# Gaurav14cs17/Bayer_Low_light_Image_Enhancement

Measured on AMD Instinct MI355X. Metric: megapixels/sec RawFormer-S 512x512 RAW->sRGB, higher is better.
Workload: dtype f32; 1 GPU; RawFormer-S(FLCA) dim=32, batch=8 of packed 4x512x512 synthetic Bayer per GPU; frames_per_gpu=8, variant=flca, weights=synthetic (seeded, random-init scale), parallelism=batch-sharded x1, device=AMD Radeon Graphics

## Files before the change

### bayer_low_light_image_enhancement_amd/build.py

```python
from __future__ import annotations

import os
import shutil
import subprocess
import sys
import tempfile
from concurrent.futures import ThreadPoolExecutor

HERE = os.path.dirname(os.path.abspath(__file__))
CSRC = os.path.join(HERE, "csrc")
LIB = os.path.join(CSRC, "librawformer_hip.so")
DIAG_LIB = os.path.join(CSRC, "librawformer_hip_diag.so")
DIAG_SOURCES = ["rf_block.hip", "rf_model.hip", "rf_gemm1x1.hip", "rf_fused.hip"]
SOURCES = ["rf_api.hip", "rf_registry.hip", "rf_model.hip", "rf_pack.hip", "rf_pointwise.hip", "rf_gemm1x1.hip",
           "rf_conv3x3.hip", "rf_attn.hip", "rf_flca.hip", "rf_fused.hip", "rf_fused_tail.hip", "rf_block.hip", "rf_harness.hip", "rf_ssim.hip", "rf_tokattn.hip", "rf_wfb.hip", "rf_upcat.hip", "rf_fft.hip", "rf_ffab.hip", "rf_truecolor.hip", "rf_multilvl.hip", "rf_train.hip", "rf_trainstep.hip", "rf_sampler.hip", "rf_mamba.hip", "rf_mamba_bwd.hip", "rf_wmb.hip"]
HEADERS = [os.path.join(CSRC, "rf_common.h"), os.path.join(CSRC, "rf_handle.h"), os.path.join(CSRC, "rf_fused_tile.h"), os.path.join(CSRC, "rf_mamba.h"), os.path.join(HERE, "..", "include", "rawformer_hip.h"),
           os.path.join(HERE, "isa_check.py")]
FLAGS = ["-O3", "-std=c++17", "-fPIC", "--offload-arch=gfx950", "-Wall", "-Wno-unused-function"]


def _hipcc() -> str:
    exe = shutil.which("hipcc") or "/opt/rocm/bin/hipcc"
    if not os.path.exists(exe):
        raise RuntimeError("hipcc not found: the RawFormer HIP library cannot be built here")
    return exe


def _run(cmd, cwd=None) -> str:
    r = subprocess.run(cmd, capture_output=True, text=True, cwd=cwd)
    if r.returncode != 0:
        raise RuntimeError("build step failed:\n" + " ".join(cmd) + "\n" + r.stdout + r.stderr)
    return r.stderr


def compile_source(src: str, obj: str, extra_flags=(), verbose: bool = False) -> int:
    from . import isa_check

    hipcc = _hipcc()
    llvm = isa_check.LLVM_BIN
    flags = [*FLAGS, *extra_flags]
    tmp = tempfile.mkdtemp(prefix="rf_build_")
    try:
        dev_s, dev_o, dev_co, fb = (os.path.join(tmp, n) for n in ("dev.s", "dev.o", "dev.co", "dev.hipfb"))
        warn = _run([hipcc, *flags, "--cuda-device-only", "-S", src, "-o", dev_s])
        text, nfix = isa_check.commute_vulnerable(open(dev_s).read())
        if nfix:
            open(dev_s, "w").write(text)
        _run([os.path.join(llvm, "clang"), "-target", "amdgcn-amd-amdhsa", "-mcpu=gfx950", "-c", dev_s, "-o", dev_o])
# ... 63 lines not shown
```

### bayer_low_light_image_enhancement_amd/csrc/rf_attn.hip

```cpp
#include "rf_common.h"

namespace rf {

static constexpr int kMaxBand = 4;
static constexpr int kRowW = kMaxBand * 16 + 2;

__host__ __device__ static inline void band_of(int tq, int C, int c, int* tklo, int* nb) {
    const int lo_ch = 16 * tq;
    const int hi_ch = (16 * tq + 15 < C - 1) ? 16 * tq + 15 : C - 1;
    const int hlo = lo_ch / c, hhi = hi_ch / c;
    const int klo = hlo * c, khi = (hhi + 1) * c - 1;
    *tklo = klo / 16;
    *nb = khi / 16 - *tklo + 1;
}

int gram_plan(int B, int C, int heads, int P, int* nslab, int* slab, size_t* partial_floats) {
    RF_CHECK_ARG(heads > 0 && C % heads == 0, "chan_attn: C=%d not divisible by heads=%d", C, heads);
    const int c = C / heads;
    RF_CHECK_ARG(c <= 64, "chan_attn: head size %d > 64 not supported", c);
    const int NTq = cdiv(C, 16);
    for (int tq = 0; tq < NTq; ++tq) {
        int tklo, nb;
        band_of(tq, C, c, &tklo, &nb);
        RF_CHECK_ARG(nb <= kMaxBand, "chan_attn: C=%d with %d heads (head size %d) needs %d key tiles per query tile, at most %d supported",
// ... 126 lines not shown
    nq += __shfl_xor(nq, 16); nq += __shfl_xor(nq, 32);
    nk += __shfl_xor(nk, 16); nk += __shfl_xor(nk, 32);
#pragma unroll
    for (int r = 0; r < 4; ++r) {
        const int row = 4 * kq + r;
#pragma unroll
        for (int t = 0; t < kMaxBand; ++t) red[wave][row][t * 16 + i] = g[t][r];
        if (row == i) {
            red[wave][row][kMaxBand * 16] = nq;
            red[wave][row][kMaxBand * 16 + 1] = nk;
        }
    }
    __syncthreads();
    float* dst = a.partial + (((size_t)b * a.nslab + slab_id) * gridDim.y + tq) * 16 * kRowW;
    for (int idx = threadIdx.x; idx < 16 * kRowW; idx += 256) {
        const int row = idx / kRowW, col = idx % kRowW;
        dst[idx] = ((red[0][row][col] + red[1][row][col]) + red[2][row][col]) + red[3][row][col];
    }
}

int launch_gram(const GramArgs& a, hipStream_t st) {
    RF_CHECK_ARG(a.B > 0 && a.B <= 65535 && a.C > 0 && a.P > 0, "gram: bad sizes");
    const int vec = (a.P % 4 == 0) && aligned16(a.q) && aligned16(a.k) && (a.bstride % 4 == 0);
    dim3 grid((unsigned)a.nslab, (unsigned)cdiv(a.C, 16), (unsigned)a.B);
    const double c = (double)a.C / a.heads;
    ProfScope prof(st, "gram_kernel", 2.0 * a.C * c * a.P * a.B, 8.0 * a.C * (double)a.P * a.B);
    RF_CHECK_ARG(a.x_hi == 0 || (a.w > 0 && a.P % a.w == 0 && a.x_lo >= 0 && a.x_lo < a.x_hi && a.x_hi <= a.w),
                 "gram: columns [%d, %d) outside the %d-wide image", a.x_lo, a.x_hi, a.w);
    if (a.x_hi > 0) gram_kernel<true><<<grid, 256, 0, st>>>(a, vec);
    else gram_kernel<false><<<grid, 256, 0, st>>>(a, vec);
    return check_launch("gram");
}

__global__ void __launch_bounds__(256) attn_fold_kernel(const float* __restrict__ partial, int nslab,
                                                        const float* __restrict__ temperature,
                                                        const float* __restrict__ w_out, float* __restrict__ wp_out,
                                                        unsigned short* __restrict__ wp3_out, int C, int heads, int log_temperature) {
    const int hd = blockIdx.x, b = blockIdx.y;
    const int c = C / heads;
    const int NT = (C + 15) >> 4;
    __shared__ float S[64][65];
    __shared__ float nq[64], nk[64];
    const float* pb = partial + (size_t)b * nslab * NT * 16 * kRowW;
    __shared__ float sub[256];
    const int nval = c * c + 2 * c;
    int RS = 256 / nval;
    if (RS < 1) RS = 1;
    if (RS > 16) RS = 16;
    for (int base = 0; base < nval; base += 256 / RS) {
        const int vi = base + threadIdx.x / RS, rs = threadIdx.x % RS;
        float s = 0.f;
        if (vi < nval && threadIdx.x / RS < 256 / RS) {
            int qch, col;
            if (vi < c * c) {
                const int ii = vi / c, jj = vi % c;
                qch = hd * c + ii;
                const int kch = hd * c + jj;
                int tklo, nb;
                band_of(qch >> 4, C, c, &tklo, &nb);
                col = ((kch >> 4) - tklo) * 16 + (kch & 15);
            } else if (vi < c * c + c) {
                qch = hd * c + (vi - c * c);
                col = kMaxBand * 16;
            } else {
                qch = hd * c + (vi - c * c - c);
                col = kMaxBand * 16 + 1;
            }
            const float* src = pb + ((size_t)(qch >> 4) * 16 + (qch & 15)) * kRowW + col;
            int sl = rs;
            for (; sl + 7 * RS < nslab; sl += 8 * RS) {
                float t[8];
#pragma unroll
                for (int u = 0; u < 8; ++u) t[u] = src[(size_t)(sl + u * RS) * NT * 16 * kRowW];
#pragma unroll
                for (int u = 0; u < 8; ++u) s += t[u];
            }
            for (; sl < nslab; sl += RS) s += src[(size_t)sl * NT * 16 * kRowW];
        }
        sub[threadIdx.x] = s;
        __syncthreads();
        if (rs == 0 && vi < nval && threadIdx.x / RS < 256 / RS) {
            float t = 0.f;
            for (int q = 0; q < RS; ++q) t += sub[threadIdx.x + q];
            if (vi < c * c) S[vi / c][vi % c] = t;
            else if (vi < c * c + c) nq[vi - c * c] = t;
            else nk[vi - c * c - c] = t;
        }
        __syncthreads();
    }
    if (threadIdx.x < c) {
        const int ii = threadIdx.x;
        const float T = log_temperature ? expf(temperature[hd]) : temperature[hd];
        const float rq = 1.0f / fmaxf(sqrtf(nq[ii]), 1e-12f);
        float m = -INFINITY;
        for (int jj = 0; jj < c; ++jj) {
            const float v = S[ii][jj] * rq * (1.0f / fmaxf(sqrtf(nk[jj]), 1e-12f)) * T;
            S[ii][jj] = v;
            m = fmaxf(m, v);
        }
        float sum = 0.f;
        for (int jj = 0; jj < c; ++jj) {
            const float e = expf(S[ii][jj] - m);
            S[ii][jj] = e;
            sum += e;
        }
        const float inv = 1.0f / sum;
        for (int jj = 0; jj < c; ++jj) S[ii][jj] *= inv;
    }
    __syncthreads();
    float* dst = wp_out + (size_t)b * NT * (C / 4) * 64;
    const int NB = (C + 31) >> 5;
    unsigned short* dst3 = wp3_out ? wp3_out + (size_t)b * NT * NB * 1536 : nullptr;
    for (int idx = threadIdx.x; idx < NT * 16 * c; idx += 256) {
        const int co = idx / c, jj = idx % c;
        float s = 0.f;
        if (co < C) {
            const float* wr = w_out + (size_t)co * C + hd * c;
            for (int ii = 0; ii < c; ++ii) s = fmaf(wr[ii], S[ii][jj], s);
        }
        const int k = hd * c + jj;
        dst[((size_t)(k >> 2) * NT + (co >> 4)) * 64 + (co & 15) + 16 * (k & 3)] = s;
        if (dst3) b3_store(dst3, NT, co, k, s);
    }
    if (dst3 && hd == heads - 1)
        for (int idx = threadIdx.x; idx < NT * 16 * (32 * NB - C); idx += 256)
            b3_store(dst3, NT, idx / (32 * NB - C), C + idx % (32 * NB - C), 0.f);
}

int launch_attn_fold(const float* partial, int nslab, const float* temperature, const float* w_out,
                     float* wp_out, void* wp3_out, int B, int C, int heads, hipStream_t st, int log_temperature) {
    RF_CHECK_ARG(C % heads == 0 && C / heads <= 64 && C % 4 == 0, "attn_fold: unsupported C=%d heads=%d", C, heads);
    ProfScope prof(st, "attn_fold_kernel", 0.0, 0.0);
    attn_fold_kernel<<<dim3((unsigned)heads, (unsigned)B), 256, 0, st>>>(partial, nslab, temperature, w_out, wp_out, (unsigned short*)wp3_out, C, heads, log_temperature);
    return check_launch("attn_fold");
}

}
```

### bayer_low_light_image_enhancement_amd/csrc/rf_fused.hip

```cpp
#include <cstdio>
#include <cstdlib>
#include "rf_common.h"
#ifdef RF_STAMP
namespace rf { __device__ unsigned long long g_stamp[16]; }
#endif
#include "rf_fused_tile.h"

namespace rf {

template <int C, int KP>
__device__ __forceinline__ void load_step_b3p(const float* __restrict__ xb, int P, int kq, const GroupGeom& g, float4 (&xh)[KP / 4]) {
#pragma unroll
    for (int s = 0; s < KP / 4; ++s) {
        const int ch = 32 * (s >> 3) + 8 * kq + (s & 7);
        xh[s] = *reinterpret_cast<const float4*>(xb + (size_t)(ch < C ? ch : 0) * P + (unsigned)g.goff);
    }
}

template <int C, int KP>
__device__ __forceinline__ void ln_step_b3p(int kq, const float* __restrict__ gam_l, const float* __restrict__ bet_l, float eps, float4 (&xh)[KP / 4]) {
    constexpr int NS = KP / 4;
    float sum[4] = {0.f, 0.f, 0.f, 0.f};
#pragma unroll
    for (int s = 0; s < NS; ++s) {
// ... 284 lines not shown
                    const int hc = 4 * s + kq, cv = 2 * C + vp * PART + hc;
                    float v[4];
                    stencil4<Edge::Dpp>(mid + hc * PSV + wave * HC + 4 * j + 4, ro, j, wd_l + cv * 9, bd_l[cv], v);
                    *reinterpret_cast<float4*>(vb + (unsigned)((vp * PART + hc) * P + yo * w + xo)) = make_float4(v[0], v[1], v[2], v[3]);
                }
            }
            STAMP(4);
        }
    }
    STAMP_FLUSH;
    __syncthreads();
    float* red = mid;
#pragma unroll
    for (int r = 0; r < NQT; ++r) {
        for (int i = tid; i < 64 * 48; i += 256) red[(i / 48) * ROWW + 16 + i % 48] = 0.f;
        float nqt = nq[r], nkt = nk[r];
        nqt += __shfl_xor(nqt, 16); nqt += __shfl_xor(nqt, 32);
        nkt += __shfl_xor(nkt, 16); nkt += __shfl_xor(nkt, 32);
#pragma unroll
        for (int q = 0; q < 4; ++q) {
            const int row = 4 * kq + q;
            float* rr = red + (wave * 16 + row) * ROWW;
            rr[j] = gq[r][q];
            if (row == j) { rr[64] = nqt; rr[65] = nkt; }
        }
        __syncthreads();
        float* dst = a.partial + (((size_t)b * a.nslab + slab) * NQT + r) * 16 * ROWW;
        for (int i = tid; i < 16 * ROWW; i += 256)
            dst[i] = ((red[i] + red[16 * ROWW + i]) + red[2 * 16 * ROWW + i]) + red[3 * 16 * ROWW + i];
        __syncthreads();
    }
}

static bool heads_fit_tiles(int C, int heads) {
    const int c = heads > 0 ? C / heads : 0;
    return heads > 0 && C % heads == 0 && c <= 16 && 16 % c == 0;
}
static bool attn_front_shape_ok(int C, int h, int w) { return C == 32 && (w % 4 == 0) && ((double)C * h * w * 4.0 < 4.0e9); }
bool fused_attn_supported(int C, int heads, int h, int w) { return heads_fit_tiles(C, heads) && attn_front_shape_ok(C, h, w); }

int fused_attn_plan(int h, int w, int* nslab, size_t* partial_floats, int B, int C) {
    const int ntiles = cdiv(w, fused::TW) * cdiv(h, fused::TH);
    int ns = cdiv(ntiles, 4);
    if (ntiles <= 256) ns = ntiles;
    if (ns < 1) ns = 1;
    *nslab = ns;
    *partial_floats = (size_t)B * ns * (C / 16) * 16 * 66;
    return RF_OK;
}

int launch_attn_front(AttnFrontArgs a, int C, hipStream_t st) {
    const int B = a.B, h = a.h, w = a.w;
    RF_CHECK_ARG(attn_front_shape_ok(C, h, w) && B <= 65535, "attn_front: unsupported shape C=%d %dx%d", C, h, w);
    RF_CHECK_ARG(aligned16(a.x) && aligned16(a.v), "attn_front: buffers must be 16-byte aligned");
    a.tiles_x = cdiv(w, fused::TW);
    a.ntiles = a.tiles_x * cdiv(h, fused::TH);
    if (!(a.yhi > 0 && a.yhi < h)) a.yhi = h;
    if (!(a.xhi > 0 && a.xhi < w)) a.xhi = w;
    const double px = (double)B * h * w;
    ProfScope prof(st, "attn_front_kernel<32>", px * (6.0 * C * C + 54.0 * C + 4.0 * C * 16), px * 8.0 * C);
    const dim3 grid((unsigned)a.nslab, (unsigned)B);
    attn_front_kernel<32><<<grid, 256, 0, st>>>(a);
    return check_launch("attn_front");
}

template <int C>
__global__ void __launch_bounds__(256, 2) attn_mid_kernel(AttnMidArgs a) {
    using namespace fused;
    constexpr int NQT = C / 16;
    constexpr int NVP = C / PART;
    constexpr int NR = NQT + NVP;
    constexpr int PSG = fused::PSG, PSV = 448, ROWW = 4 * 16 + 2;
    constexpr int NF4 = PART * HR * (HC / 4);
    constexpr int FPT = (NF4 + 255) / 256;
    constexpr unsigned OOB = 0x80000000u;
    __shared__ __attribute__((aligned(16))) float mid[PART * PSG + 8];
    __shared__ float wd_l[3 * C * 9], bd_l[3 * C];

    const int tid = threadIdx.x, lane = tid & 63, wave = tid >> 6;
    const int j = lane & 15, kq = lane >> 4;
    const int slab = blockIdx.x, b = blockIdx.y;
    const int h = a.h, w = a.w, P = h * w;
    const float* qb = a.qkv + (size_t)b * 3 * C * P;
    float* vb = a.v + (size_t)b * C * P;
    for (int i = tid; i < 3 * C * 9; i += 256) wd_l[i] = a.wd[i];
    for (int i = tid; i < 3 * C; i += 256) bd_l[i] = a.bd[i];

    int pk[FPT];
#pragma unroll
    for (int i = 0; i < FPT; ++i) {
        const int e = tid + 256 * i;
        const int pl = e / (HR * (HC / 4)), rem = e % (HR * (HC / 4));
        pk[i] = e < NF4 ? (pl << 16) | ((rem / (HC / 4)) << 8) | (rem % (HC / 4)) : -1;
    }
    const int tiles_y = a.ntiles / a.tiles_x;
    const int per = (a.ntiles + a.nslab - 1) / a.nslab;
    unsigned voff[FPT];
    int pend_ys = 0;
    bool pend_full = true;
    auto plan_tile = [&](int tile, bool full) {
        const int2 o = tile_origin(tile, tiles_y);
        const int x0 = o.x, y0 = o.y;
        pend_ys = y0 % HR; pend_full = full;
#pragma unroll
        for (int i = 0; i < FPT; ++i) {
            int e = pk[i];
            asm volatile("" : "+v"(e));
            const int r = (e >> 8) & 255;
            const int y = y0 - 1 + r, x = x0 - 4 + 4 * (e & 255);
            const bool ok = e >= 0 && (full || r >= 2) && (unsigned)y < (unsigned)h && (unsigned)x < (unsigned)w;
            voff[i] = ok ? (unsigned)((y * w + x) * 4) : OOB;
        }
    };
    float4 stg[FPT];
    auto load_round = [&](int rd) {
        const bool gram = rd < NQT;
        const size_t base = gram ? (size_t)16 * rd * P : (size_t)(2 * C + PART * (rd - NQT)) * P;
        const size_t span = (gram ? (size_t)(C + 16) : (size_t)PART) * P, rest = (size_t)3 * C * P - base;
        const __amdgpu_buffer_rsrc_t rs = __builtin_amdgcn_make_buffer_rsrc(
            const_cast<float*>(qb) + base, 0, (int)((span < rest ? span : rest) * 4), 0x00020000);
        const unsigned kjump = gram ? (unsigned)((C - 16) * P) * 4u : 0u;
#pragma unroll
        for (int i = 0; i < FPT; ++i) {
            const int pl = pk[i] >> 16;
            const unsigned off = voff[i] + (unsigned)pl * (unsigned)P * 4u + (pl >= 16 ? kjump : 0u);
            typedef unsigned u32x4_t __attribute__((ext_vector_type(4)));
            const u32x4_t v4 = __builtin_amdgcn_raw_buffer_load_b128(rs, (int)off, 0, 0);
            stg[i] = make_float4(__uint_as_float(v4.x), __uint_as_float(v4.y), __uint_as_float(v4.z), __uint_as_float(v4.w));
        }
    };
    auto store_round = [&](int rd) {
        const int PSX = rd < NQT ? PSG : PSV;
#pragma unroll
        for (int i = 0; i < FPT; ++i) {
            int e = pk[i];
            asm volatile("" : "+v"(e));
            const int r = (e >> 8) & 255;
            const int slot = pend_ys + r - (pend_ys + r >= HR ? HR : 0);
            if (e >= 0 && (pend_full || r >= 2)) *reinterpret_cast<float4*>(mid + (e >> 16) * PSX + slot * HC + 4 * (e & 255)) = stg[i];
        }
    };

    const int t_begin = slab * per;
    if (t_begin >= a.ntiles) {
        if ((int)blockIdx.z == 0)
            for (int i = tid; i < NQT * 16 * ROWW; i += 256) a.partial[((size_t)b * a.nslab + slab) * NQT * 16 * ROWW + i] = 0.f;
        return;
    }
    const int ntw = (t_begin + per < a.ntiles) ? per : a.ntiles - t_begin;
    f32x4 gq = {0.f, 0.f, 0.f, 0.f};
    float nq = 0.f, nk = 0.f;
    const int rd_lo = (int)blockIdx.z * NR / a.rgroups, rd_hi = ((int)blockIdx.z + 1) * NR / a.rgroups;
    plan_tile(t_begin, true);
    load_round(rd_lo);
    __syncthreads();
    for (int rd = rd_lo; rd < rd_hi; ++rd) {
        for (int ti = 0; ti < ntw; ++ti) {
            const int tile = t_begin + ti;
            const int2 o = tile_origin(tile, tiles_y);
            const int x0 = o.x, y0 = o.y;
            const int yo = y0 + wave;
            lds_barrier();
            store_round(rd);
            int ro[3];
#pragma unroll
            for (int dy = 0; dy < 3; ++dy) {
                const int sl = pend_ys + wave + dy;
                ro[dy] = (sl - (sl >= HR ? HR : 0)) * HC;
            }
            if (ti + 1 < ntw) {
                plan_tile(tile + 1, (tile + 1) % tiles_y == 0);
                load_round(rd);
            } else if (rd + 1 < rd_hi) {
                plan_tile(t_begin, true);
                load_round(rd + 1);
            }
            lds_barrier();
            if (rd < NQT) {
                const int cq = 16 * rd + j, ck = C + 16 * rd + j;
#pragma unroll 1
                for (int st = 0; st < 4; ++st) {
                    const int xo = x0 + 16 * st + 4 * kq;
                    const bool ok = yo >= a.ylo && yo < a.yhi && xo >= a.xlo && xo < a.xhi;
                    float qa[4], kb[4];
                    stencil4<Edge::Wide>(mid + j * PSG + 16 * st + 4 * kq + 4, ro, j, wd_l + cq * 9, bd_l[cq], qa);
                    stencil4<Edge::Wide>(mid + (16 + j) * PSG + 16 * st + 4 * kq + 4, ro, j, wd_l + ck * 9, bd_l[ck], kb);
#pragma unroll
                    for (int m = 0; m < 4; ++m) {
                        const float qv = ok ? qa[m] : 0.f, kv = ok ? kb[m] : 0.f;
                        gq = __builtin_amdgcn_mfma_f32_16x16x4f32(qv, kv, gq, 0, 0, 0);
                        nq = fmaf(qv, qv, nq);
                        nk = fmaf(kv, kv, nk);
                    }
                }
            } else {
                const int vp = rd - NQT, xo = x0 + 4 * j;
                if (yo < h && xo < w) {
#pragma unroll
                    for (int s = 0; s < PART / 4; ++s) {
                        const int hc = 4 * s + kq, cv = 2 * C + vp * PART + hc;
                        float v[4];
                        stencil4<Edge::Dpp>(mid + hc * PSV + 4 * j + 4, ro, j, wd_l + cv * 9, bd_l[cv], v);
                        *reinterpret_cast<float4*>(vb + (size_t)(vp * PART + hc) * P + (size_t)yo * w + xo) = make_float4(v[0], v[1], v[2], v[3]);
                    }
                }
            }
        }
        if (rd < NQT) {
            __syncthreads();
            float* red = mid;
            for (int i = tid; i < 64 * 48; i += 256) red[(i / 48) * ROWW + 16 + i % 48] = 0.f;
            int kq_ = kq;
            asm volatile("" : "+v"(kq_));
            float nqt = nq, nkt = nk;
            nqt += __shfl_xor(nqt, 16); nqt += __shfl_xor(nqt, 32);
            nkt += __shfl_xor(nkt, 16); nkt += __shfl_xor(nkt, 32);
#pragma unroll
            for (int q = 0; q < 4; ++q) {
                const int row = 4 * kq_ + q;
                float* rr = red + (wave * 16 + row) * ROWW;
                rr[j] = gq[q];
                if (row == j) { rr[64] = nqt; rr[65] = nkt; }
            }
            __syncthreads();
            float* dst = a.partial + (((size_t)b * a.nslab + slab) * NQT + rd) * 16 * ROWW;
            for (int i = tid; i < 16 * ROWW; i += 256)
                dst[i] = ((red[i] + red[16 * ROWW + i]) + red[2 * 16 * ROWW + i]) + red[3 * 16 * ROWW + i];
            gq = (f32x4){0.f, 0.f, 0.f, 0.f}; nq = 0.f; nk = 0.f;
        }
    }
}

int attn_mid_plan(int h, int w, int* nslab, size_t* partial_floats, int B, int C) {
    const int ntiles = cdiv(w, fused::TW) * cdiv(h, fused::TH);
    int per = ntiles / 64;
    if (per < 1) per = 1;
    if (per > 8) per = 8;
    *nslab = cdiv(ntiles, per);
    *partial_floats = (size_t)B * *nslab * (C / 16) * 16 * 66;
    return RF_OK;
}

static bool attn_mid_shape_ok(int C, int h, int w) {
    return (C == 64 || C == 128) && (w % 4 == 0) && ((double)(C + 16) * h * w * 4.0 < 2.0e9);
}
bool attn_mid_supported(int C, int heads, int h, int w) { return heads_fit_tiles(C, heads) && attn_mid_shape_ok(C, h, w); }

int launch_attn_mid(AttnMidArgs a, int C, hipStream_t st) {
    const int B = a.B, h = a.h, w = a.w;
    RF_CHECK_ARG(attn_mid_shape_ok(C, h, w) && B <= 65535, "attn_mid: unsupported shape C=%d %dx%d", C, h, w);
    RF_CHECK_ARG(aligned16(a.qkv) && aligned16(a.v), "attn_mid: buffers must be 16-byte aligned");
    a.tiles_x = cdiv(w, fused::TW);
    a.ntiles = a.tiles_x * cdiv(h, fused::TH);
    if (!(a.yhi > 0 && a.yhi < h)) a.yhi = h;
    if (!(a.xhi > 0 && a.xhi < w)) a.xhi = w;
    a.rgroups = ((long)a.nslab * B < 256) ? 3 : 1;
    const double px = (double)B * h * w;
    ProfScope prof(st, C == 64 ? "attn_mid_kernel<64>" : "attn_mid_kernel<128>", px * (54.0 * C + 4.0 * C * 16), px * 16.0 * C);
    const dim3 grid((unsigned)a.nslab, (unsigned)B, (unsigned)a.rgroups);
    if (C == 64) attn_mid_kernel<64><<<grid, 256, 0, st>>>(a);
    else attn_mid_kernel<128><<<grid, 256, 0, st>>>(a);
    return check_launch("attn_mid");
}

#ifdef RF_STAMP
extern "C" int rf_debug_stamps(unsigned long long* out8) {
    unsigned long long z[16] = {0};
    if (hipMemcpyFromSymbol(out8, HIP_SYMBOL(g_stamp), 8 * sizeof(unsigned long long)) != hipSuccess) return -1;
    return hipMemcpyToSymbol(HIP_SYMBOL(g_stamp), z, sizeof(z)) == hipSuccess ? 0 : -1;
}
#endif

}
```

### bayer_low_light_image_enhancement_amd/csrc/rf_fused_tile.h

```cpp
#pragma once
#include "rf_common.h"

namespace rf {

#ifdef RF_STAMP
#define STAMP_DECL unsigned long long st_prev = __builtin_amdgcn_s_memtime(), st_acc[8] = {0, 0, 0, 0, 0, 0, 0, 0};
#define STAMP(i) do { __builtin_amdgcn_sched_barrier(0); unsigned long long t_ = __builtin_amdgcn_s_memtime(); st_acc[i] += t_ - st_prev; st_prev = t_; __builtin_amdgcn_sched_barrier(0); } while (0)
#define STAMP_FLUSH do { if ((threadIdx.x & 63) == 0) for (int i_ = 0; i_ < 8; ++i_) atomicAdd(&g_stamp[i_], st_acc[i_]); } while (0)
#else
#define STAMP_DECL
#define STAMP(i)
#define STAMP_FLUSH
#endif

__device__ __forceinline__ void lds_barrier() {
    asm volatile("s_waitcnt lgkmcnt(0)" ::: "memory");
    __builtin_amdgcn_s_barrier();
    asm volatile("" ::: "memory");
}

namespace fused {
constexpr int TH = 4, TW = 64;
constexpr int HR = TH + 2;
constexpr int HC = 72;
constexpr int NG = HR * (HC / 4);
constexpr int GPW = NG / 4;
constexpr int GPW8 = 14;
constexpr int PART = 32;
constexpr int PSG = 456;
}

struct GroupGeom {
    int lds_off;
    int goff;
    bool valid;
};
template <int G>
__device__ __forceinline__ GroupGeom group_geom(int wave, int st, int j, int y0, int x0, int h, int w) {
    using namespace fused;
    GroupGeom g;
    const int gi = wave * G + st * 16 + j;
    const bool in_step = j < G - st * 16 && (NG % G == 0 || gi < NG);
    const int row = gi / (HC / 4), cg = gi % (HC / 4);
    const int y = y0 - 1 + row, x = x0 - 4 + 4 * cg;
    g.valid = in_step && y >= 0 && y < h && x >= 0 && x < w;
    g.lds_off = in_step ? row * HC + 4 * cg : -1;
    g.goff = g.valid ? y * w + x : 0;
    return g;
}

struct TileRange { int tiles_y, begin, end; };
// ... 292 lines not shown
```

Baseline: 1093 MP/s.

## Move attn_mid to its own file with column-major tile walk and rewrite attn_fold

Moves the attention-mid kernel into its own source file and reworks its tile iteration. Tiles now advance down columns with a rolling row ring in LDS, so each step loads only the new rows, and per-lane load offsets are precomputed once using buffer out-of-bounds masking. Depthwise weights are hoisted per round. The fold kernel may now launch with 1024 threads, unrolls the slab reduction 16-wide, and stages w_out rows in dynamic shared memory. This adds complexity and register pressure in the mid kernel.

```diff
diff --git a/bayer_low_light_image_enhancement_amd/build.py b/bayer_low_light_image_enhancement_amd/build.py
--- a/bayer_low_light_image_enhancement_amd/build.py
+++ b/bayer_low_light_image_enhancement_amd/build.py
@@ -13,7 +13,7 @@
 DIAG_LIB = os.path.join(CSRC, "librawformer_hip_diag.so")
 DIAG_SOURCES = ["rf_block.hip", "rf_model.hip", "rf_gemm1x1.hip", "rf_fused.hip"]
 SOURCES = ["rf_api.hip", "rf_registry.hip", "rf_model.hip", "rf_pack.hip", "rf_pointwise.hip", "rf_gemm1x1.hip",
-           "rf_conv3x3.hip", "rf_attn.hip", "rf_flca.hip", "rf_fused.hip", "rf_fused_tail.hip", "rf_block.hip", "rf_harness.hip", "rf_ssim.hip", "rf_tokattn.hip", "rf_wfb.hip", "rf_upcat.hip", "rf_fft.hip", "rf_ffab.hip", "rf_truecolor.hip", "rf_multilvl.hip", "rf_train.hip", "rf_trainstep.hip", "rf_sampler.hip", "rf_mamba.hip", "rf_mamba_bwd.hip", "rf_wmb.hip"]
+           "rf_conv3x3.hip", "rf_attn.hip", "rf_flca.hip", "rf_fused.hip", "rf_fused_tail.hip", "rf_attn_mid.hip", "rf_block.hip", "rf_harness.hip", "rf_ssim.hip", "rf_tokattn.hip", "rf_wfb.hip", "rf_upcat.hip", "rf_fft.hip", "rf_ffab.hip", "rf_truecolor.hip", "rf_multilvl.hip", "rf_train.hip", "rf_trainstep.hip", "rf_sampler.hip", "rf_mamba.hip", "rf_mamba_bwd.hip", "rf_wmb.hip"]
 HEADERS = [os.path.join(CSRC, "rf_common.h"), os.path.join(CSRC, "rf_handle.h"), os.path.join(CSRC, "rf_fused_tile.h"), os.path.join(CSRC, "rf_mamba.h"), os.path.join(HERE, "..", "include", "rawformer_hip.h"),
            os.path.join(HERE, "isa_check.py")]
 FLAGS = ["-O3", "-std=c++17", "-fPIC", "--offload-arch=gfx950", "-Wall", "-Wno-unused-function"]
diff --git a/bayer_low_light_image_enhancement_amd/csrc/rf_attn.hip b/bayer_low_light_image_enhancement_amd/csrc/rf_attn.hip
--- a/bayer_low_light_image_enhancement_amd/csrc/rf_attn.hip
+++ b/bayer_low_light_image_enhancement_amd/csrc/rf_attn.hip
@@ -182,25 +182,33 @@
     return check_launch("gram");
 }
 
-__global__ void __launch_bounds__(256) attn_fold_kernel(const float* __restrict__ partial, int nslab,
-                                                        const float* __restrict__ temperature,
-                                                        const float* __restrict__ w_out, float* __restrict__ wp_out,
-                                                        unsigned short* __restrict__ wp3_out, int C, int heads, int log_temperature) {
+constexpr int kFoldThreads = 1024;
+constexpr int kFoldStage = 8192;
+static int fold_threads(int c) { return c * c + 2 * c > 256 ? kFoldThreads : 256; }
+__host__ __device__ static inline int fold_stage(int NT, int c) { return NT * 16 * c < kFoldStage ? NT * 16 * c : kFoldStage; }
+__global__ void __launch_bounds__(kFoldThreads) attn_fold_kernel(const float* __restrict__ partial, int nslab,
+                                                                 const float* __restrict__ temperature,
+                                                                 const float* __restrict__ w_out, float* __restrict__ wp_out,
+                                                                 unsigned short* __restrict__ wp3_out, int C, int heads, int log_temperature) {
     const int hd = blockIdx.x, b = blockIdx.y;
     const int c = C / heads;
     const int NT = (C + 15) >> 4;
     __shared__ float S[64][65];
     __shared__ float nq[64], nk[64];
     const float* pb = partial + (size_t)b * nslab * NT * 16 * kRowW;
-    __shared__ float sub[256];
+    extern __shared__ float fold_dyn[];
+    const int nthr = (int)blockDim.x;
+    float* sub = fold_dyn;
     const int nval = c * c + 2 * c;
     int RS = 256 / nval;
     if (RS < 1) RS = 1;
     if (RS > 16) RS = 16;
-    for (int base = 0; base < nval; base += 256 / RS) {
+    const int vpp = nthr / RS;
+    for (int base = 0; base < nval; base += vpp) {
         const int vi = base + threadIdx.x / RS, rs = threadIdx.x % RS;
+        const bool mine = vi < nval && (int)threadIdx.x / RS < vpp;
         float s = 0.f;
-        if (vi < nval && threadIdx.x / RS < 256 / RS) {
+        if (mine) {
             int qch, col;
             if (vi < c * c) {
                 const int ii = vi / c, jj = vi % c;
@@ -217,19 +225,27 @@
                 col = kMaxBand * 16 + 1;
             }
             const float* src = pb + ((size_t)(qch >> 4) * 16 + (qch & 15)) * kRowW + col;
+            const size_t sstride = (size_t)NT * 16 * kRowW;
             int sl = rs;
-            for (; sl + 7 * RS < nslab; sl += 8 * RS) {
-                float t[8];
-#pragma unroll
-                for (int u = 0; u < 8; ++u) t[u] = src[(size_t)(sl + u * RS) * NT * 16 * kRowW];
-#pragma unroll
-                for (int u = 0; u < 8; ++u) s += t[u];
-            }
-            for (; sl < nslab; sl += RS) s += src[(size_t)sl * NT * 16 * kRowW];
+            for (; sl + 15 * RS < nslab; sl += 16 * RS) {
+                float t[16];
+#pragma unroll
+                for (int u = 0; u < 16; ++u) t[u] = src[(size_t)(sl + u * RS) * sstride];
+#pragma unroll
+                for (int u = 0; u < 16; ++u) s += t[u];
+            }
+            for (; sl + 3 * RS < nslab; sl += 4 * RS) {
+                float t[4];
+#pragma unroll
+                for (int u = 0; u < 4; ++u) t[u] = src[(size_t)(sl + u * RS) * sstride];
+#pragma unroll
+                for (int u = 0; u < 4; ++u) s += t[u];
+            }
+            for (; sl < nslab; sl += RS) s += src[(size_t)sl * sstride];
         }
         sub[threadIdx.x] = s;
         __syncthreads();
-        if (rs == 0 && vi < nval && threadIdx.x / RS < 256 / RS) {
+        if (rs == 0 && mine) {
             float t = 0.f;
             for (int q = 0; q < RS; ++q) t += sub[threadIdx.x + q];
             if (vi < c * c) S[vi / c][vi % c] = t;
@@ -261,19 +277,30 @@
     float* dst = wp_out + (size_t)b * NT * (C / 4) * 64;
     const int NB = (C + 31) >> 5;
     unsigned short* dst3 = wp3_out ? wp3_out + (size_t)b * NT * NB * 1536 : nullptr;
-    for (int idx = threadIdx.x; idx < NT * 16 * c; idx += 256) {
-        const int co = idx / c, jj = idx % c;
-        float s = 0.f;
-        if (co < C) {
-            const float* wr = w_out + (size_t)co * C + hd * c;
-            for (int ii = 0; ii < c; ++ii) s = fmaf(wr[ii], S[ii][jj], s);
-        }
-        const int k = hd * c + jj;
-        dst[((size_t)(k >> 2) * NT + (co >> 4)) * 64 + (co & 15) + 16 * (k & 3)] = s;
-        if (dst3) b3_store(dst3, NT, co, k, s);
+    float* wl = fold_dyn + nthr;
+    const int rows = fold_stage(NT, c) / c;
+    for (int co0 = 0; co0 < NT * 16; co0 += rows) {
+        const int nrow = NT * 16 - co0 < rows ? NT * 16 - co0 : rows;
+        __syncthreads();
+        for (int idx = threadIdx.x; idx < nrow * c; idx += nthr) {
+            const int co = co0 + idx / c;
+            wl[idx] = co < C ? w_out[(size_t)co * C + hd * c + idx % c] : 0.f;
+        }
+        __syncthreads();
+        for (int idx = threadIdx.x; idx < nrow * c; idx += nthr) {
+            const int co = co0 + idx / c, jj = idx % c;
+            float s = 0.f;
+            if (co < C) {
+                const float* wr = wl + (idx - jj);
+                for (int ii = 0; ii < c; ++ii) s = fmaf(wr[ii], S[ii][jj], s);
+            }
+            const int k = hd * c + jj;
+            dst[((size_t)(k >> 2) * NT + (co >> 4)) * 64 + (co & 15) + 16 * (k & 3)] = s;
+            if (dst3) b3_store(dst3, NT, co, k, s);
+        }
     }
     if (dst3 && hd == heads - 1)
-        for (int idx = threadIdx.x; idx < NT * 16 * (32 * NB - C); idx += 256)
+        for (int idx = threadIdx.x; idx < NT * 16 * (32 * NB - C); idx += nthr)
             b3_store(dst3, NT, idx / (32 * NB - C), C + idx % (32 * NB - C), 0.f);
 }
 
@@ -281,7 +308,8 @@
                      float* wp_out, void* wp3_out, int B, int C, int heads, hipStream_t st, int log_temperature) {
     RF_CHECK_ARG(C % heads == 0 && C / heads <= 64 && C % 4 == 0, "attn_fold: unsupported C=%d heads=%d", C, heads);
     ProfScope prof(st, "attn_fold_kernel", 0.0, 0.0);
-    attn_fold_kernel<<<dim3((unsigned)heads, (unsigned)B), 256, 0, st>>>(partial, nslab, temperature, w_out, wp_out, (unsigned short*)wp3_out, C, heads, log_temperature);
+    const int c = C / heads, nthr = fold_threads(c);
+    attn_fold_kernel<<<dim3((unsigned)heads, (unsigned)B), nthr, (size_t)(nthr + fold_stage((C + 15) >> 4, c)) * sizeof(float), st>>>(partial, nslab, temperature, w_out, wp_out, (unsigned short*)wp3_out, C, heads, log_temperature);
     return check_launch("attn_fold");
 }
 
diff --git a/bayer_low_light_image_enhancement_amd/csrc/rf_attn_mid.hip b/bayer_low_light_image_enhancement_amd/csrc/rf_attn_mid.hip
--- /dev/null
+++ b/bayer_low_light_image_enhancement_amd/csrc/rf_attn_mid.hip
@@ -0,0 +1,285 @@
+#include <cstdio>
+#include <cstdlib>
+#include "rf_common.h"
+#include "rf_fused_tile.h"
+
+namespace rf {
+
+template <int C>
+__global__ void __launch_bounds__(256, 2) attn_mid_kernel(AttnMidArgs a) {
+    using namespace fused;
+    constexpr int NQT = C / 16;
+    constexpr int NVP = C / PART;
+    constexpr int NR = NQT + NVP;
+    constexpr int PSG = fused::PSG, PSV = 448, ROWW = 4 * 16 + 2;
+    constexpr int G4 = HC / 4;
+    constexpr int PE = PART * 2 * G4;
+    constexpr int KP = (PE + 255) / 256;
+    static_assert(PE == 4 * 256 + 128 && KP == 5, "the last element of a pair belongs to waves 0 and 1");
+    constexpr unsigned OOB = 0x80000000u;
+    __shared__ __attribute__((aligned(16))) float mid[PART * PSG + 8];
+    __shared__ float wd_l[3 * C * 9], bd_l[3 * C];
+
+    const int tid = threadIdx.x, lane = tid & 63, wave = tid >> 6;
+    const int j = lane & 15, kq = lane >> 4;
+    const int slab = blockIdx.x, b = blockIdx.y;
+    const int h = a.h, w = a.w, P = h * w;
+    const float* qb = a.qkv + (size_t)b * 3 * C * P;
+    float* vb = a.v + (size_t)b * C * P;
+    for (int i = tid; i < 3 * C * 9; i += 256) wd_l[i] = a.wd[i];
+    for (int i = tid; i < 3 * C; i += 256) bd_l[i] = a.bd[i];
+
+    const int tiles_y = a.ntiles / a.tiles_x;
+    const int per = (a.ntiles + a.nslab - 1) / a.nslab;
+    const int t_begin = slab * per;
+    if (t_begin >= a.ntiles) {
+        if ((int)blockIdx.z == 0)
+            for (int i = tid; i < NQT * 16 * ROWW; i += 256) a.partial[((size_t)b * a.nslab + slab) * NQT * 16 * ROWW + i] = 0.f;
+        return;
+    }
+    const int ntw = (t_begin + per < a.ntiles) ? per : a.ntiles - t_begin;
+    const int rd_lo = (int)blockIdx.z * NR / a.rgroups, rd_hi = ((int)blockIdx.z + 1) * NR / a.rgroups;
+
+    const unsigned w4 = (unsigned)w * 4u, w16 = w4 * 4u;
+    const unsigned kjump = (unsigned)((C - 16) * P) * 4u;
+    const int wave_u = __builtin_amdgcn_readfirstlane(wave);
+    const bool wave_lo = wave_u < 2;
+    unsigned rel[KP];
+    float* lp[KP];
+    int key[KP];
+    {
+        const bool gram = rd_lo < NQT;
+#pragma unroll
+        for (int k = 0; k < KP; ++k) {
+            const int e = tid + 256 * k;
+            const int pl = e / (2 * G4), rem = e % (2 * G4), sub = rem / G4, g = rem % G4;
+            const bool there = e < PE;
+            key[k] = there ? g | (pl << 5) | (sub << 10) : 31;
+            rel[k] = there ? (unsigned)sub * w4 + 16u * (unsigned)g + (unsigned)pl * (unsigned)P * 4u + (gram && pl >= 16 ? kjump : 0u) : 0u;
+            lp[k] = mid + (there ? pl * (gram ? PSG : PSV) + sub * HC + 4 * g : 0);
+        }
+    }
+    auto set_column = [&](int x0) {
+        const int glo = x0 == 0 ? 1 : 0, gtop = ((w - x0) >> 2) + 1, gn = (gtop < G4 ? gtop : G4) - glo;
+#pragma unroll
+        for (int k = 0; k < KP; ++k) rel[k] = (rel[k] & ~OOB) | ((unsigned)((key[k] & 31) - glo) < (unsigned)gn ? 0u : OOB);
+    };
+    auto to_v_rounds = [&]() {
+#pragma unroll
+        for (int k = 0; k < KP; ++k) {
+            const int pl = (key[k] >> 5) & 31;
+            rel[k] -= pl >= 16 ? kjump : 0u;
+            lp[k] -= pl * (PSG - PSV);
+        }
+    };
+    const size_t P16 = (size_t)16 * P, PV = (size_t)PART * P, base_v0 = (size_t)2 * C * P, span_g = (size_t)(C + 16) * P, total = (size_t)3 * C * P;
+    size_t r_base = rd_lo < NQT ? (size_t)rd_lo * P16 : base_v0 + (size_t)(rd_lo - NQT) * PV;
+    auto next_base = [&](int rd_next) { return rd_next < NQT ? r_base + P16 : rd_next == NQT ? base_v0 : r_base + PV; };
+    auto round_rsrc = [&](size_t base, bool gram) {
+        const size_t span = gram ? span_g : PV, rest = total - base;
+        return __builtin_amdgcn_make_buffer_rsrc(const_cast<float*>(qb) + base, 0, (int)((span < rest ? span : rest) * 4), 0x00020000);
+    };
+
+    int n_tx = t_begin / tiles_y, n_ty = t_begin % tiles_y;
+    const int tx0 = n_tx, ty0 = n_ty, k0 = (2 * ty0) % 3;
+    const unsigned tb0 = ((unsigned)(ty0 * TH) * (unsigned)w + (unsigned)(tx0 * TW)) * 4u;
+    int n_k = k0;
+    unsigned n_tb = tb0;
+    bool n_full = true;
+    int col_tx = n_tx;
+    const int ro_top = wave_u * HC, ro_0 = ((2 * k0 + wave_u) % HR) * HC;
+    int n_ro = ro_0;
+    float* const v_lane = vb + (size_t)kq * P + (size_t)wave * w + 4 * j;
+    const size_t P4 = (size_t)4 * P;
+    size_t v_round = rd_lo > NQT ? (size_t)(rd_lo - NQT) * PV : 0;
+    int vw_off = (2 * C + (rd_lo > NQT ? (rd_lo - NQT) * PART : 0) + kq) * 9, vb_off = 2 * C + (rd_lo > NQT ? (rd_lo - NQT) * PART : 0) + kq;
+    int gw_off = (16 * rd_lo + j) * 9;
+    float* dstp = a.partial + (((size_t)b * a.nslab + slab) * NQT + (rd_lo < NQT ? rd_lo : 0)) * 16 * ROWW;
+    set_column(n_tx * TW);
+
+    float4 stg[3][KP];
+    typedef unsigned u32x4_t __attribute__((ext_vector_type(4)));
+    auto forget = [](float4& v) { asm volatile("" : "=v"(v.x), "=v"(v.y), "=v"(v.z), "=v"(v.w)); };
+    auto load_tile = [&](const __amdgpu_buffer_rsrc_t rs) {
+#pragma unroll
+        for (int p = 0; p < 3; ++p) {
+            const int d = p - n_k + (p < n_k ? 3 : 0);
+            if (n_full || d != 0) {
+                const int ya = n_ty * TH - 1 + 2 * d;
+                const bool va = (unsigned)ya < (unsigned)h, vb2 = (unsigned)(ya + 1) < (unsigned)h;
+                const unsigned rowbase = n_tb - w4 - 16u + (d == 0 ? 0u : d == 1 ? 2u * w4 : w16);
+                if (va && vb2) {
+#pragma unroll
+                    for (int k = 0; k < KP; ++k)
+                        if (k < KP - 1 || wave_lo) {
+                            const u32x4_t v4 = __builtin_amdgcn_raw_buffer_load_b128(rs, (int)(rel[k] + rowbase), 0, 0);
+                            stg[p][k] = make_float4(__uint_as_float(v4.x), __uint_as_float(v4.y), __uint_as_float(v4.z), __uint_as_float(v4.w));
+                        } else forget(stg[p][k]);
+                } else {
+                    const unsigned ia = va ? 0u : OOB, ib = vb2 ? 0u : OOB;
+#pragma unroll
+                    for (int k = 0; k < KP; ++k)
+                        if (k < KP - 1 || wave_lo) {
+                            const unsigned off = (rel[k] | ((key[k] & 1024) ? ib : ia)) + rowbase;
+                            const u32x4_t v4 = __builtin_amdgcn_raw_buffer_load_b128(rs, (int)off, 0, 0);
+                            stg[p][k] = make_float4(__uint_as_float(v4.x), __uint_as_float(v4.y), __uint_as_float(v4.z), __uint_as_float(v4.w));
+                        } else forget(stg[p][k]);
+                }
+            } else {
+#pragma unroll
+                for (int k = 0; k < KP; ++k) forget(stg[p][k]);
+            }
+        }
+    };
+
+    const int ntw1 = ntw - 1;
+    f32x4 gq = {0.f, 0.f, 0.f, 0.f};
+    float nq = 0.f, nk = 0.f;
+    load_tile(round_rsrc(r_base, rd_lo < NQT));
+    __syncthreads();
+    for (int rd = rd_lo; rd < rd_hi; ++rd) {
+        const __amdgpu_buffer_rsrc_t rs = round_rsrc(r_base, rd < NQT);
+        float wq[9], wk[9], bq = 0.f, bk = 0.f;
+        if (rd < NQT) {
+            const int cq = 16 * rd + j;
+#pragma unroll
+            for (int t = 0; t < 9; ++t) { wq[t] = wd_l[gw_off + t]; wk[t] = wd_l[gw_off + 9 * C + t]; }
+            bq = bd_l[cq]; bk = bd_l[C + cq];
+            gw_off += 16 * 9;
+        } else {
+#pragma unroll
+            for (int t = 0; t < 9; ++t) wq[t] = wk[t] = 0.f;
+        }
+        for (int ti = 0; ti < ntw; ++ti) {
+            const int x0 = n_tx * TW, y0 = n_ty * TH;
+            const int yo = y0 + wave;
+            const int c_k = n_k, c_ro = n_ro;
+            const bool c_full = n_full;
+            const size_t c_px = n_tb >> 2;
+            lds_barrier();
+#pragma unroll
+            for (int p = 0; p < 3; ++p)
+                if (c_full || p != c_k) {
+#pragma unroll
+                    for (int k = 0; k < KP; ++k)
+                        if (k < KP - 1 || wave_lo) *reinterpret_cast<float4*>(lp[k] + 2 * p * HC) = stg[p][k];
+                }
+            int ro[3];
+#pragma unroll
+            for (int dy = 0; dy < 3; ++dy) {
+                const int r = c_ro + dy * HC;
+                ro[dy] = r - (r >= HR * HC ? HR * HC : 0);
+            }
+            if (ti < ntw1) {
+                ++n_ty; n_k = n_k == 0 ? 2 : n_k - 1; n_tb += w16; n_full = false;
+                n_ro += 4 * HC; n_ro -= n_ro >= HR * HC ? HR * HC : 0;
+                if (n_ty == tiles_y) { n_ty = 0; ++n_tx; n_k = 0; n_tb = (unsigned)(n_tx * TW) * 4u; n_full = true; n_ro = ro_top; }
+                if (n_tx != col_tx) { col_tx = n_tx; set_column(n_tx * TW); }
+                load_tile(rs);
+            } else if (rd + 1 < rd_hi) {
+                n_tx = tx0; n_ty = ty0; n_k = k0; n_tb = tb0; n_full = true; n_ro = ro_0;
+                if (n_tx != col_tx) { col_tx = n_tx; set_column(n_tx * TW); }
+                if (rd + 1 == NQT) to_v_rounds();
+                load_tile(round_rsrc(next_base(rd + 1), rd + 1 < NQT));
+            }
+            lds_barrier();
+            if (rd < NQT) {
+#pragma unroll 1
+                for (int st = 0; st < 4; ++st) {
+                    const int xo = x0 + 16 * st + 4 * kq;
+                    const bool ok = yo >= a.ylo && yo < a.yhi && xo >= a.xlo && xo < a.xhi;
+                    float qa[4], kb[4];
+                    stencil4<Edge::Wide>(mid + j * PSG + 16 * st + 4 * kq + 4, ro, j, wq, bq, qa);
+                    stencil4<Edge::Wide>(mid + (16 + j) * PSG + 16 * st + 4 * kq + 4, ro, j, wk, bk, kb);
+#pragma unroll
+                    for (int m = 0; m < 4; ++m) {
+                        const float qv = ok ? qa[m] : 0.f, kv = ok ? kb[m] : 0.f;
+                        gq = __builtin_amdgcn_mfma_f32_16x16x4f32(qv, kv, gq, 0, 0, 0);
+                        nq = fmaf(qv, qv, nq);
+                        nk = fmaf(kv, kv, nk);
+                    }
+                }
+            } else {
+                const int xo = x0 + 4 * j;
+                if (yo < h && xo < w) {
+                    size_t so = v_round + c_px;
+#pragma unroll
+                    for (int s = 0; s < PART / 4; ++s) {
+                        const int hc = 4 * s + kq;
+                        float v[4];
+                        stencil4<Edge::Dpp>(mid + hc * PSV + 4 * j + 4, ro, j, wd_l + vw_off + 36 * s, bd_l[vb_off + 4 * s], v);
+                        *reinterpret_cast<float4*>(v_lane + so) = make_float4(v[0], v[1], v[2], v[3]);
+                        so += P4;
+                    }
+                }
+            }
+        }
+        if (rd < NQT) {
+            __syncthreads();
+            float* red = mid;
+            int kq_ = kq;
+            asm volatile("" : "+v"(kq_));
+            float nqt = nq, nkt = nk;
+            nqt += __shfl_xor(nqt, 16); nqt += __shfl_xor(nqt, 32);
+            nkt += __shfl_xor(nkt, 16); nkt += __shfl_xor(nkt, 32);
+#pragma unroll
+            for (int q = 0; q < 4; ++q) {
+                const int row = 4 * kq_ + q;
+                float* rr = red + (wave * 16 + row) * ROWW;
+                rr[j] = gq[q];
+                if (row == j) { rr[64] = nqt; rr[65] = nkt; }
+            }
+            __syncthreads();
+            float* dst = dstp;
+            dstp += 16 * ROWW;
+            auto sum4 = [&](int i) { return ((red[i] + red[16 * ROWW + i]) + red[2 * 16 * ROWW + i]) + red[3 * 16 * ROWW + i]; };
+            int t_ = tid;
+            asm volatile("" : "+v"(t_));
+            const int ri = (t_ >> 4) * ROWW + (t_ & 15);
+            dst[ri] = sum4(ri);
+            dst[ri + 16] = 0.f; dst[ri + 32] = 0.f; dst[ri + 48] = 0.f;
+            if (t_ < 32) {
+                const int si = (t_ >> 1) * ROWW + 64 + (t_ & 1);
+                dst[si] = sum4(si);
+            }
+            gq = (f32x4){0.f, 0.f, 0.f, 0.f}; nq = 0.f; nk = 0.f;
+        } else {
+            v_round += PV; vw_off += PART * 9; vb_off += PART;
+        }
+        r_base = next_base(rd + 1);
+    }
+}
+
+int attn_mid_plan(int h, int w, int* nslab, size_t* partial_floats, int B, int C) {
+    const int ntiles = cdiv(w, fused::TW) * cdiv(h, fused::TH);
+    int per = ntiles / 64;
+    if (per < 1) per = 1;
+    if (per > 8) per = 8;
+    *nslab = cdiv(ntiles, per);
+    *partial_floats = (size_t)B * *nslab * (C / 16) * 16 * 66;
+    return RF_OK;
+}
+
+static bool attn_mid_shape_ok(int C, int h, int w) {
+    return (C == 64 || C == 128) && (w % 4 == 0) && ((double)(C + 16) * h * w * 4.0 < 2.0e9);
+}
+bool attn_mid_supported(int C, int heads, int h, int w) { return heads_fit_tiles(C, heads) && attn_mid_shape_ok(C, h, w); }
+
+int launch_attn_mid(AttnMidArgs a, int C, hipStream_t st) {
+    const int B = a.B, h = a.h, w = a.w;
+    RF_CHECK_ARG(attn_mid_shape_ok(C, h, w) && B <= 65535, "attn_mid: unsupported shape C=%d %dx%d", C, h, w);
+    RF_CHECK_ARG(aligned16(a.qkv) && aligned16(a.v), "attn_mid: buffers must be 16-byte aligned");
+    a.tiles_x = cdiv(w, fused::TW);
+    a.ntiles = a.tiles_x * cdiv(h, fused::TH);
+    if (!(a.yhi > 0 && a.yhi < h)) a.yhi = h;
+    if (!(a.xhi > 0 && a.xhi < w)) a.xhi = w;
+    a.rgroups = ((long)a.nslab * B < 256) ? 3 : 1;
+    const double px = (double)B * h * w;
+    ProfScope prof(st, C == 64 ? "attn_mid_kernel<64>" : "attn_mid_kernel<128>", px * (54.0 * C + 4.0 * C * 16), px * 16.0 * C);
+    const dim3 grid((unsigned)a.nslab, (unsigned)B, (unsigned)a.rgroups);
+    if (C == 64) attn_mid_kernel<64><<<grid, 256, 0, st>>>(a);
+    else attn_mid_kernel<128><<<grid, 256, 0, st>>>(a);
+    return check_launch("attn_mid");
+}
+
+}
diff --git a/bayer_low_light_image_enhancement_amd/csrc/rf_fused.hip b/bayer_low_light_image_enhancement_amd/csrc/rf_fused.hip
--- a/bayer_low_light_image_enhancement_amd/csrc/rf_fused.hip
+++ b/bayer_low_light_image_enhancement_amd/csrc/rf_fused.hip
@@ -340,10 +340,6 @@
     }
 }
 
-static bool heads_fit_tiles(int C, int heads) {
-    const int c = heads > 0 ? C / heads : 0;
-    return heads > 0 && C % heads == 0 && c <= 16 && 16 % c == 0;
-}
 static bool attn_front_shape_ok(int C, int h, int w) { return C == 32 && (w % 4 == 0) && ((double)C * h * w * 4.0 < 4.0e9); }
 bool fused_attn_supported(int C, int heads, int h, int w) { return heads_fit_tiles(C, heads) && attn_front_shape_ok(C, h, w); }
 
@@ -372,205 +368,6 @@
     return check_launch("attn_front");
 }
 
-template <int C>
-__global__ void __launch_bounds__(256, 2) attn_mid_kernel(AttnMidArgs a) {
-    using namespace fused;
-    constexpr int NQT = C / 16;
-    constexpr int NVP = C / PART;
-    constexpr int NR = NQT + NVP;
-    constexpr int PSG = fused::PSG, PSV = 448, ROWW = 4 * 16 + 2;
-    constexpr int NF4 = PART * HR * (HC / 4);
-    constexpr int FPT = (NF4 + 255) / 256;
-    constexpr unsigned OOB = 0x80000000u;
-    __shared__ __attribute__((aligned(16))) float mid[PART * PSG + 8];
-    __shared__ float wd_l[3 * C * 9], bd_l[3 * C];
-
-    const int tid = threadIdx.x, lane = tid & 63, wave = tid >> 6;
-    const int j = lane & 15, kq = lane >> 4;
-    const int slab = blockIdx.x, b = blockIdx.y;
-    const int h = a.h, w = a.w, P = h * w;
-    const float* qb = a.qkv + (size_t)b * 3 * C * P;
-    float* vb = a.v + (size_t)b * C * P;
-    for (int i = tid; i < 3 * C * 9; i += 256) wd_l[i] = a.wd[i];
-    for (int i = tid; i < 3 * C; i += 256) bd_l[i] = a.bd[i];
-
-    int pk[FPT];
-#pragma unroll
-    for (int i = 0; i < FPT; ++i) {
-        const int e = tid + 256 * i;
-        const int pl = e / (HR * (HC / 4)), rem = e % (HR * (HC / 4));
-        pk[i] = e < NF4 ? (pl << 16) | ((rem / (HC / 4)) << 8) | (rem % (HC / 4)) : -1;
-    }
-    const int tiles_y = a.ntiles / a.tiles_x;
-    const int per = (a.ntiles + a.nslab - 1) / a.nslab;
-    unsigned voff[FPT];
-    int pend_ys = 0;
-    bool pend_full = true;
-    auto plan_tile = [&](int tile, bool full) {
-        const int2 o = tile_origin(tile, tiles_y);
-        const int x0 = o.x, y0 = o.y;
-        pend_ys = y0 % HR; pend_full = full;
-#pragma unroll
-        for (int i = 0; i < FPT; ++i) {
-            int e = pk[i];
-            asm volatile("" : "+v"(e));
-            const int r = (e >> 8) & 255;
-            const int y = y0 - 1 + r, x = x0 - 4 + 4 * (e & 255);
-            const bool ok = e >= 0 && (full || r >= 2) && (unsigned)y < (unsigned)h && (unsigned)x < (unsigned)w;
-            voff[i] = ok ? (unsigned)((y * w + x) * 4) : OOB;
-        }
-    };
-    float4 stg[FPT];
-    auto load_round = [&](int rd) {
-        const bool gram = rd < NQT;
-        const size_t base = gram ? (size_t)16 * rd * P : (size_t)(2 * C + PART * (rd - NQT)) * P;
-        const size_t span = (gram ? (size_t)(C + 16) : (size_t)PART) * P, rest = (size_t)3 * C * P - base;
-        const __amdgpu_buffer_rsrc_t rs = __builtin_amdgcn_make_buffer_rsrc(
-            const_cast<float*>(qb) + base, 0, (int)((span < rest ? span : rest) * 4), 0x00020000);
-        const unsigned kjump = gram ? (unsigned)((C - 16) * P) * 4u : 0u;
-#pragma unroll
-        for (int i = 0; i < FPT; ++i) {
-            const int pl = pk[i] >> 16;
-            const unsigned off = voff[i] + (unsigned)pl * (unsigned)P * 4u + (pl >= 16 ? kjump : 0u);
-            typedef unsigned u32x4_t __attribute__((ext_vector_type(4)));
-            const u32x4_t v4 = __builtin_amdgcn_raw_buffer_load_b128(rs, (int)off, 0, 0);
-            stg[i] = make_float4(__uint_as_float(v4.x), __uint_as_float(v4.y), __uint_as_float(v4.z), __uint_as_float(v4.w));
-        }
-    };
-    auto store_round = [&](int rd) {
-        const int PSX = rd < NQT ? PSG : PSV;
-#pragma unroll
-        for (int i = 0; i < FPT; ++i) {
-            int e = pk[i];
-            asm volatile("" : "+v"(e));
-            const int r = (e >> 8) & 255;
-            const int slot = pend_ys + r - (pend_ys + r >= HR ? HR : 0);
-            if (e >= 0 && (pend_full || r >= 2)) *reinterpret_cast<float4*>(mid + (e >> 16) * PSX + slot * HC + 4 * (e & 255)) = stg[i];
-        }
-    };
-
-    const int t_begin = slab * per;
-    if (t_begin >= a.ntiles) {
-        if ((int)blockIdx.z == 0)
-            for (int i = tid; i < NQT * 16 * ROWW; i += 256) a.partial[((size_t)b * a.nslab + slab) * NQT * 16 * ROWW + i] = 0.f;
-        return;
-    }
-    const int ntw = (t_begin + per < a.ntiles) ? per : a.ntiles - t_begin;
-    f32x4 gq = {0.f, 0.f, 0.f, 0.f};
-    float nq = 0.f, nk = 0.f;
-    const int rd_lo = (int)blockIdx.z * NR / a.rgroups, rd_hi = ((int)blockIdx.z + 1) * NR / a.rgroups;
-    plan_tile(t_begin, true);
-    load_round(rd_lo);
-    __syncthreads();
-    for (int rd = rd_lo; rd < rd_hi; ++rd) {
-        for (int ti = 0; ti < ntw; ++ti) {
-            const int tile = t_begin + ti;
-            const int2 o = tile_origin(tile, tiles_y);
-            const int x0 = o.x, y0 = o.y;
-            const int yo = y0 + wave;
-            lds_barrier();
-            store_round(rd);
-            int ro[3];
-#pragma unroll
-            for (int dy = 0; dy < 3; ++dy) {
-                const int sl = pend_ys + wave + dy;
-                ro[dy] = (sl - (sl >= HR ? HR : 0)) * HC;
-            }
-            if (ti + 1 < ntw) {
-                plan_tile(tile + 1, (tile + 1) % tiles_y == 0);
-                load_round(rd);
-            } else if (rd + 1 < rd_hi) {
-                plan_tile(t_begin, true);
-                load_round(rd + 1);
-            }
-            lds_barrier();
-            if (rd < NQT) {
-                const int cq = 16 * rd + j, ck = C + 16 * rd + j;
-#pragma unroll 1
-                for (int st = 0; st < 4; ++st) {
-                    const int xo = x0 + 16 * st + 4 * kq;
-                    const bool ok = yo >= a.ylo && yo < a.yhi && xo >= a.xlo && xo < a.xhi;
-                    float qa[4], kb[4];
-                    stencil4<Edge::Wide>(mid + j * PSG + 16 * st + 4 * kq + 4, ro, j, wd_l + cq * 9, bd_l[cq], qa);
-                    stencil4<Edge::Wide>(mid + (16 + j) * PSG + 16 * st + 4 * kq + 4, ro, j, wd_l + ck * 9, bd_l[ck], kb);
-#pragma unroll
-                    for (int m = 0; m < 4; ++m) {
-                        const float qv = ok ? qa[m] : 0.f, kv = ok ? kb[m] : 0.f;
-                        gq = __builtin_amdgcn_mfma_f32_16x16x4f32(qv, kv, gq, 0, 0, 0);
-                        nq = fmaf(qv, qv, nq);
-                        nk = fmaf(kv, kv, nk);
-                    }
-                }
-            } else {
-                const int vp = rd - NQT, xo = x0 + 4 * j;
-                if (yo < h && xo < w) {
-#pragma unroll
-                    for (int s = 0; s < PART / 4; ++s) {
-                        const int hc = 4 * s + kq, cv = 2 * C + vp * PART + hc;
-                        float v[4];
-                        stencil4<Edge::Dpp>(mid + hc * PSV + 4 * j + 4, ro, j, wd_l + cv * 9, bd_l[cv], v);
-                        *reinterpret_cast<float4*>(vb + (size_t)(vp * PART + hc) * P + (size_t)yo * w + xo) = make_float4(v[0], v[1], v[2], v[3]);
-                    }
-                }
-            }
-        }
-        if (rd < NQT) {
-            __syncthreads();
-            float* red = mid;
-            for (int i = tid; i < 64 * 48; i += 256) red[(i / 48) * ROWW + 16 + i % 48] = 0.f;
-            int kq_ = kq;
-            asm volatile("" : "+v"(kq_));
-            float nqt = nq, nkt = nk;
-            nqt += __shfl_xor(nqt, 16); nqt += __shfl_xor(nqt, 32);
-            nkt += __shfl_xor(nkt, 16); nkt += __shfl_xor(nkt, 32);
-#pragma unroll
-            for (int q = 0; q < 4; ++q) {
-                const int row = 4 * kq_ + q;
-                float* rr = red + (wave * 16 + row) * ROWW;
-                rr[j] = gq[q];
-                if (row == j) { rr[64] = nqt; rr[65] = nkt; }
-            }
-            __syncthreads();
-            float* dst = a.partial + (((size_t)b * a.nslab + slab) * NQT + rd) * 16 * ROWW;
-            for (int i = tid; i < 16 * ROWW; i += 256)
-                dst[i] = ((red[i] + red[16 * ROWW + i]) + red[2 * 16 * ROWW + i]) + red[3 * 16 * ROWW + i];
-            gq = (f32x4){0.f, 0.f, 0.f, 0.f}; nq = 0.f; nk = 0.f;
-        }
-    }
-}
-
-int attn_mid_plan(int h, int w, int* nslab, size_t* partial_floats, int B, int C) {
-    const int ntiles = cdiv(w, fused::TW) * cdiv(h, fused::TH);
-    int per = ntiles / 64;
-    if (per < 1) per = 1;
-    if (per > 8) per = 8;
-    *nslab = cdiv(ntiles, per);
-    *partial_floats = (size_t)B * *nslab * (C / 16) * 16 * 66;
-    return RF_OK;
-}
-
-static bool attn_mid_shape_ok(int C, int h, int w) {
-    return (C == 64 || C == 128) && (w % 4 == 0) && ((double)(C + 16) * h * w * 4.0 < 2.0e9);
-}
-bool attn_mid_supported(int C, int heads, int h, int w) { return heads_fit_tiles(C, heads) && attn_mid_shape_ok(C, h, w); }
-
-int launch_attn_mid(AttnMidArgs a, int C, hipStream_t st) {
-    const int B = a.B, h = a.h, w = a.w;
-    RF_CHECK_ARG(attn_mid_shape_ok(C, h, w) && B <= 65535, "attn_mid: unsupported shape C=%d %dx%d", C, h, w);
-    RF_CHECK_ARG(aligned16(a.qkv) && aligned16(a.v), "attn_mid: buffers must be 16-byte aligned");
-    a.tiles_x = cdiv(w, fused::TW);
-    a.ntiles = a.tiles_x * cdiv(h, fused::TH);
-    if (!(a.yhi > 0 && a.yhi < h)) a.yhi = h;
-    if (!(a.xhi > 0 && a.xhi < w)) a.xhi = w;
-    a.rgroups = ((long)a.nslab * B < 256) ? 3 : 1;
-    const double px = (double)B * h * w;
-    ProfScope prof(st, C == 64 ? "attn_mid_kernel<64>" : "attn_mid_kernel<128>", px * (54.0 * C + 4.0 * C * 16), px * 16.0 * C);
-    const dim3 grid((unsigned)a.nslab, (unsigned)B, (unsigned)a.rgroups);
-    if (C == 64) attn_mid_kernel<64><<<grid, 256, 0, st>>>(a);
-    else attn_mid_kernel<128><<<grid, 256, 0, st>>>(a);
-    return check_launch("attn_mid");
-}
-
 #ifdef RF_STAMP
 extern "C" int rf_debug_stamps(unsigned long long* out8) {
     unsigned long long z[16] = {0};
diff --git a/bayer_low_light_image_enhancement_amd/csrc/rf_fused_tile.h b/bayer_low_light_image_enhancement_amd/csrc/rf_fused_tile.h
--- a/bayer_low_light_image_enhancement_amd/csrc/rf_fused_tile.h
+++ b/bayer_low_light_image_enhancement_amd/csrc/rf_fused_tile.h
@@ -17,6 +17,11 @@
     asm volatile("s_waitcnt lgkmcnt(0)" ::: "memory");
     __builtin_amdgcn_s_barrier();
     asm volatile("" ::: "memory");
+}
+
+static inline bool heads_fit_tiles(int C, int heads) {
+    const int c = heads > 0 ? C / heads : 0;
+    return c > 0 && C % heads == 0 && c <= 16 && 16 % c == 0;
 }
 
 namespace fused {
```

New measurement: 1107 MP/s (median of 6 runs). 1.2% higher.
